# solislemuslab/BayesianNetworkRegression.jl

Measured on AMD Instinct MI355X. Metric: Gibbs iterations/sec (all chains), higher is better.
Workload: dtype f64; 1 GPU; synthetic n=500 V=100 (q=5050) R=7, 8 chains total, 8 per GPU; chains_total=8, chains_per_gpu=8, seed=20240501

## Files before the change

### bayesiannetworkregression.jl_amd/_capi.py

```python
import ctypes as C
import os

import numpy as np

from ._build import LIB

BNR_OK, BNR_ERR_BAD_ARG, BNR_ERR_HIP, BNR_ERR_CHOLESKY, BNR_ERR_SAMPLER = 0, 1, 2, 3, 4
BNR_ERR_SAMPLER_CAP = BNR_ERR_SAMPLER
ERRORS = {1: "bad argument", 2: "HIP error", 3: "Cholesky failed after jitter", 4: "sampler attempt cap"}


class BnrError(RuntimeError):
    def __init__(self, code, msg):
        super().__init__("libbnr_hip: %s (status %d: %s)" % (msg, code, ERRORS.get(code, "?")))
        self.code = code


class Hyper(C.Structure):
    _fields_ = [(k, C.c_double) for k in ("eta", "zeta", "iota", "aDelta", "bDelta", "nu")]


PROGRESS_CB = C.CFUNCTYPE(None, C.c_void_p, C.c_int64)
ALLGATHER_CB = C.CFUNCTYPE(C.c_int, C.c_void_p, C.POINTER(C.c_double), C.POINTER(C.c_double), C.c_int64)

# ... 36 lines not shown
    "bnr_chain_fetch": (C.c_int, [C.c_void_p, C.c_int32, C.c_int32, C.c_int32, C.c_int32] + [_dp] * 11),
    "bnr_chain_load": (C.c_int, [C.c_void_p, C.c_int32, C.c_int32, C.c_int32, C.c_int32] + [_dp] * 11),
    "bnr_chain_move_rows": (C.c_int, [C.c_void_p, C.c_int32, C.c_int32, C.c_int32]),
    "bnr_chain_resize": (C.c_int, [C.c_void_p, C.c_int32]),
    "bnr_chain_rhat_stats": (C.c_int, [C.c_void_p, C.c_int32, C.c_int32, _dp]),
    "bnr_chain_summary": (C.c_int, [C.c_void_p, C.c_int32, C.c_int32, C.c_int32, C.c_int32, _dp, _dp, _dp, _dp]),
    "bnr_chain_predict": (C.c_int, [C.c_void_p, C.c_int32, C.c_int32, C.c_int32, _dp, C.c_int32, _dp, C.c_int32, C.c_int32] + [_dp] * 5),
    "bnr_chain_predict_from_matrices": (C.c_int, [C.c_void_p, C.c_int32, C.c_int32, C.c_int32, C.POINTER(C.c_void_p), C.c_int32, _dp, C.c_int32,
                                                  C.c_int32] + [_dp] * 5),
    "bnr_chain_loglik_stats": (C.c_int, [C.c_void_p, C.c_int32, C.c_int32, _dp, _dp]),
    "bnr_chain_loo": (C.c_int, [C.c_void_p, C.c_int32, C.c_int32, _dp, _dp, _dp, _dp]),
    "bnr_psis_loo": (C.c_int, [C.c_int32, C.c_int32, C.c_int32, _dp, _dp, _dp, _dp, _dp]),
    "bnr_chains_summary": (C.c_int, [C.POINTER(C.c_void_p), C.c_int32, C.c_int32, C.c_int32, C.c_int32, C.c_int32, _dp, _dp, _dp, _dp]),
    "bnr_chains_predict": (C.c_int, [C.POINTER(C.c_void_p), C.c_int32, C.c_int32, C.c_int32, C.c_int32, _dp, C.c_int32, _dp, C.c_int32, C.c_int32]
                           + [_dp] * 5 + [C.c_uint64] + [_dp] * 3),
    "bnr_chains_predict_from_matrices": (C.c_int, [C.POINTER(C.c_void_p), C.c_int32, C.c_int32, C.c_int32, C.c_int32, C.POINTER(C.c_void_p), C.c_int32,
                                                   _dp, C.c_int32, C.c_int32] + [_dp] * 5 + [C.c_uint64] + [_dp] * 3),
    "bnr_chains_loglik_stats": (C.c_int, [C.POINTER(C.c_void_p), C.c_int32, C.c_int32, C.c_int32, _dp, _dp, _dp]),
    "bnr_chains_loo": (C.c_int, [C.POINTER(C.c_void_p), C.c_int32, C.c_int32, C.c_int32, _dp, _dp, _dp, _dp]),
    "bnr_chain_loo_predict": (C.c_int, [C.c_void_p, C.c_int32, C.c_int32, _dp, C.c_double, C.c_double] + [_dp] * 8),
    "bnr_chains_loo_predict": (C.c_int, [C.POINTER(C.c_void_p), C.c_int32, C.c_int32, C.c_int32, _dp, C.c_double, C.c_double] + [_dp] * 8),
    "bnr_psis_weights": (C.c_int, [C.c_int32, C.c_int32, C.c_int32, _dp, _dp, _dp, _dp, _dp]),
    "bnr_chain_rank_diag": (C.c_int, [C.c_void_p, C.c_int32, C.c_int32, C.c_int32] + [_dp] * 6),
    "bnr_chains_rank_diag": (C.c_int, [C.POINTER(C.c_void_p), C.c_int32, C.c_int32, C.c_int32, C.c_int32] + [_dp] * 6),
    "bnr_rank_normalize": (C.c_int, [C.c_int32, C.c_int32, C.c_int32, _dp, _dp, _dp]),
    "bnr_host_ndtri": (C.c_double, [C.c_double]),
    "bnr_chain_hdi": (C.c_int, [C.c_void_p, C.c_int32, C.c_int32, C.c_int32, _dp] + [_dp] * 5),
    "bnr_chains_hdi": (C.c_int, [C.POINTER(C.c_void_p), C.c_int32, C.c_int32, C.c_int32, C.c_int32, _dp] + [_dp] * 5),
    "bnr_hdi": (C.c_int, [C.c_int32, C.c_int32, C.c_int32, _dp, C.c_int32, _dp] + [_dp] * 5),
    "bnr_comm_unique_id": (C.c_int, [C.POINTER(UniqueId)]),
    "bnr_comm_create_rccl": (C.c_int, [C.POINTER(UniqueId), C.c_int32, C.c_int32, C.c_int32, C.POINTER(C.c_void_p)]),
    "bnr_comm_create_callback": (C.c_int, [C.c_int32, C.c_int32, ALLGATHER_CB, C.c_void_p, C.POINTER(C.c_void_p)]),
    "bnr_comm_destroy": (C.c_int, [C.c_void_p]),
    "bnr_comm_allgather": (C.c_int, [C.c_void_p, _dp, _dp, C.c_int64]),
    "bnr_comm_info": (C.c_int, [C.c_void_p] + [C.POINTER(C.c_int32)] * 5),
    "bnr_rhat": (C.c_int, [C.POINTER(C.c_void_p), C.c_int32, C.c_int32, C.c_void_p, C.c_int32, C.c_int32, _dp, _dp]),
    "bnr_rhat_from_stats": (C.c_int, [_dp, C.c_int32, C.c_int32, C.c_int32, _dp]),
    "bnr_chain_ess_stats": (C.c_int, [C.c_void_p, C.c_int32, C.c_int32, C.c_int32, _dp]),
    "bnr_ess_from_stats": (C.c_int, [_dp, C.c_int32, C.c_int32, C.c_int32, C.c_int32, _dp]),
    "bnr_chain_counters": (C.c_int, [C.c_void_p, C.POINTER(C.c_int64)]),
    "bnr_chain_set_profiling": (C.c_int, [C.c_void_p, C.c_int32]),
    "bnr_chain_last_timing": (C.c_int, [C.c_void_p, C.c_int32, C.POINTER(C.c_double), C.POINTER(C.c_int64)]),
    "bnr_chain_set_option": (C.c_int, [C.c_void_p, C.c_char_p, C.c_int64]),
    "bnr_chain_debug_read": (C.c_int, [C.c_void_p, C.POINTER(C.c_uint64), C.c_int32]),
    "bnr_chain_debug_copy": (C.c_int, [C.c_void_p, C.c_int32, _dp, C.c_int64]),
    "bnr_chain_debug_dims": (C.c_int, [C.c_void_p, C.POINTER(C.c_int32)]),
    "bnr_chain_debug_time_gram": (C.c_int, [C.c_void_p, C.c_int32, C.POINTER(C.c_double)]),
    "bnr_debug_set_exp": (C.c_int, [C.c_int32, C.c_int32]),
    "bnr_host_philox": (None, [C.POINTER(C.c_uint32), C.POINTER(C.c_uint32), C.POINTER(C.c_uint32)]),
    "bnr_host_uniform2": (None, [C.c_uint64, C.c_uint32, C.c_uint32, C.c_uint32, C.c_uint32, C.POINTER(C.c_double)]),
    "bnr_host_normal": (C.c_double, [C.c_uint64, C.c_uint32, C.c_uint32, C.c_uint32, C.c_uint32]),
    "bnr_host_gamma": (C.c_double, [C.c_uint64, C.c_double, C.c_uint32, C.c_uint32, C.c_uint32]),
    "bnr_host_gig": (C.c_double, [C.c_uint64, C.c_double, C.c_double, C.c_double, C.c_uint32, C.c_uint32]),
    "bnr_host_edge_index": (C.c_int32, [C.c_int32, C.c_int32, C.c_int32]),
    "bnr_host_xi_weight": (C.c_double, [C.c_double, C.c_double, C.c_double]),
    "bnr_host_pred_noise": (None, [C.c_uint64, C.c_uint32, C.c_uint32, C.c_uint32, C.c_uint32, _dp]),
    "bnr_host_gram_plan": (C.c_int, [C.c_int32, C.c_int32, C.c_int32, C.POINTER(C.c_int32)]),
}
for _u in ("tau2", "u_xi", "gamma", "D", "theta", "Delta", "M", "mu", "Lambda", "pi"):
    _SIGS["bnr_update_" + _u] = (C.c_int, [C.c_void_p, C.c_int32, C.c_int64])

EXPORTS = sorted(_SIGS)


_foreign_hip = None


def _mapped(needle):
    out = []
    try:
        with open("/proc/self/maps") as f:
            for line in f:
                parts = line.split()
                if len(parts) >= 6 and needle in os.path.basename(parts[5]) and parts[5] not in out:
                    out.append(parts[5])
    except OSError:
        pass
    return out


def lib():
    global _lib
    if _lib is None:
        if not os.path.exists(LIB):
            raise ImportError("libbnr_hip.so is missing at %s -- build it with `python -c 'import __graft_entry__ as g; "
                              "g.build()'` (hipcc --offload-arch=gfx950); there is no CPU fallback" % LIB)
        before = _mapped("libamdhip64")
        L = C.CDLL(LIB)
        after = _mapped("libamdhip64")
        foreign = [p_ for p_ in before if not os.path.realpath(p_).startswith(os.path.realpath(os.environ.get("ROCM_PATH", "/opt/rocm")))]
        global _foreign_hip
        if foreign and after == before and not os.environ.get("BNR_ALLOW_FOREIGN_HIP"):
            _foreign_hip = ("libbnr_hip.so was loaded after another HIP runtime (%s) and is bound to it instead of %s/lib: load the library "
                            "(bnr_amd._capi.lib(), or create the chains) BEFORE importing torch, or set BNR_ALLOW_FOREIGN_HIP=1 to run on the "
                            "foreign runtime" % (", ".join(foreign), os.environ.get("ROCM_PATH", "/opt/rocm")))
        for name, (res, args) in _SIGS.items():
            f = getattr(L, name)
            f.restype = res
            f.argtypes = args
        _lib = L
    return _lib


def check(code):
    if code != BNR_OK:
        raise BnrError(code, lib().bnr_last_error().decode())
# ... 631 lines not shown
```

### bayesiannetworkregression.jl_amd/csrc/bnr_hip.hip

```cpp
#include "bnr_internal.h"
#include "bnr_kernels.h"

#include <dlfcn.h>

#include <cmath>
#include <cstdio>
#include <mutex>

static thread_local std::string g_err;
int fail(int code, const std::string &msg) { g_err = msg; return code; }
static thread_local hipError_t g_noted = hipSuccess;
static thread_local const char *g_noted_what = nullptr;
#define HIPNOTE(expr)                                                                                  \
    do {                                                                                               \
        hipError_t _e = (expr);                                                                        \
        if (_e != hipSuccess && g_noted == hipSuccess) { g_noted = _e; g_noted_what = #expr; }         \
    } while (0)

template <typename T>
static int dev_alloc(bnr_chain *c, T **p, size_t count, bool zero = true)
{
    void *q = nullptr;
    HIPCHK(hipMalloc(&q, std::max<size_t>(count, 1) * sizeof(T)));
    if (zero) HIPCHK(hipMemsetAsync(q, 0, std::max<size_t>(count, 1) * sizeof(T), c->x.stream));
// ... 18 lines not shown
    std::lock_guard<std::mutex> lock(mu);
    if ((int)done.size() <= device) done.resize(device + 1, 0);
    if (done[device]) return BNR_OK;
    const int big = 124 * 1024;
    const void *fns[] = {(const void *)&k_tail<bnr_one>, (const void *)&k_tail<bnr_many>, (const void *)&k_backproj<bnr_one>,
                         (const void *)&k_backproj<bnr_many>, (const void *)&k_solve_a4<bnr_one>, (const void *)&k_solve_a4<bnr_many>,
                         (const void *)&k_xpass_group, (const void *)&k_node<bnr_one>, (const void *)&k_node<bnr_many>};
    for (const void *f : fns) HIPCHK(hipFuncSetAttribute(f, hipFuncAttributeMaxDynamicSharedMemorySize, big));
    if (int rc = late_kernels_lds_attributes(big)) return rc;
    done[device] = 1;
    return BNR_OK;
}

extern "C" {

static int exec_init(bnr_exec &x, int device, int nb, const bnr_dev *shape);
static void exec_free(bnr_exec &x);
static int sync_dev(bnr_chain *c);

int bnr_abi_version(void) { return BNR_ABI_VERSION; }
const char *bnr_last_error(void) { return g_err.c_str(); }
int bnr_device_synchronize(int32_t device)
{
    HIPCHK(hipSetDevice(device));
    HIPCHK(hipDeviceSynchronize());
    return BNR_OK;
}
int bnr_runtime_version(int *version)
{
    if (!version) return fail(BNR_ERR_BAD_ARG, "version is NULL");
    HIPCHK(hipRuntimeGetVersion(version));
    return BNR_OK;
}
int bnr_device_count(int *count)
{
    if (!count) return fail(BNR_ERR_BAD_ARG, "count is NULL");
    HIPCHK(hipGetDeviceCount(count));
    return BNR_OK;
}

void bnr_host_philox(const uint32_t ctr[4], const uint32_t key[2], uint32_t out[4])
{
    bnr_u4 r = bnr_philox4x32_10(ctr[0], ctr[1], ctr[2], ctr[3], key[0], key[1]);
    out[0] = r.x; out[1] = r.y; out[2] = r.z; out[3] = r.w;
}
void bnr_host_uniform2(uint64_t seed, uint32_t it, uint32_t site, uint32_t elem, uint32_t att, double out[2])
{ bnr_draw2(seed, it, site, elem, att, out[0], out[1]); }
double bnr_host_normal(uint64_t seed, uint32_t it, uint32_t site, uint32_t elem, uint32_t att)
{ return bnr_normal(seed, it, site, elem, att); }
double bnr_host_gamma(uint64_t seed, double shape, uint32_t it, uint32_t site, uint32_t elem)
{ int cap = 0; return bnr_gamma(seed, shape, it, site, elem, &cap); }
double bnr_host_gig(uint64_t seed, double lambda, double chi, double psi, uint32_t it, uint32_t elem)
{ int cap = 0; return bnr_gig(seed, lambda, chi, psi, it, elem, &cap); }
int32_t bnr_host_edge_index(int32_t V, int32_t l, int32_t k)
{ return l >= k ? bnr_edge_index(V, l, k) : bnr_edge_index(V, k, l); }
double bnr_host_xi_weight(double lt, double lb, double Delta)
{ return bnr_xi_weight_ref(lt, lb, Delta); }

static int alloc_trace(bnr_chain *c, int tot, double **out)
{
    void *p = nullptr;
    size_t bytes = (size_t)(tot + 2) * c->d.rowlen * sizeof(double);
    HIPCHK(hipMalloc(&p, bytes));
    HIPCHK(hipMemsetAsync(p, 0, bytes, c->x.stream));
    *out = (double *)p;
    c->trace_bytes = bytes;
    return BNR_OK;
}

extern "C++" size_t dtype_size(int t) { return t == BNR_U8 ? 1 : (t == BNR_I32 || t == BNR_F32) ? 4 : 8; }
extern "C++" template <typename T>
static void launch_x_convert_as(const void *raw, bool mats, int rows, const bnr_dev &d, int ld, double *Xd, unsigned char *X8, int *not_bytes, hipStream_t st)
{
    hipLaunchKernelGGL(k_x_convert<T>, dim3((rows + 63) / 64, std::min(d.q, 65535)), dim3(64), 0, st, (const T *)raw, mats, rows, d.V, d.q, ld, d.ek, d.el, Xd, X8,
                       not_bytes);
}
extern "C++" void launch_x_convert(int dtype, const void *raw, bool mats, int rows, const bnr_dev &d, int ld, double *Xd, unsigned char *X8, int *not_bytes, hipStream_t st)
{
    switch (dtype) {
    case BNR_U8:  launch_x_convert_as<uint8_t>(raw, mats, rows, d, ld, Xd, X8, not_bytes, st); break;
    case BNR_I32: launch_x_convert_as<int32_t>(raw, mats, rows, d, ld, Xd, X8, not_bytes, st); break;
    case BNR_I64: launch_x_convert_as<int64_t>(raw, mats, rows, d, ld, Xd, X8, not_bytes, st); break;
    case BNR_F32: launch_x_convert_as<float>(raw, mats, rows, d, ld, Xd, nullptr, not_bytes, st); break;
    default:      launch_x_convert_as<double>(raw, mats, rows, d, ld, Xd, nullptr, not_bytes, st); break;
    }
}
static int upload_x(bnr_chain *c, const x_source &src, double *Xd, unsigned char *X8, int *not_bytes_dev)
{
    const bnr_dev &d = c->d;
    const size_t es = dtype_size(src.dtype);
    if (!src.mats && src.dtype == BNR_F64) {
        HIPCHK(hipMemcpy2D(Xd, (size_t)d.n_pad * sizeof(double), src.X, (size_t)d.n * sizeof(double), (size_t)d.n * sizeof(double), d.q, hipMemcpyHostToDevice));
        return BNR_OK;
    }
    const size_t count = src.mats ? (size_t)d.n * d.V * d.V : (size_t)d.n * d.q;
    void *raw = nullptr;
    HIPCHK(hipMalloc(&raw, count * es));
    hipError_t e = hipSuccess;
    if (src.mats) {
        for (int i = 0; i < d.n && e == hipSuccess; ++i) {
            if (!src.mats[i]) { (void)hipFree(raw); return fail(BNR_ERR_BAD_ARG, "NULL adjacency matrix"); }
            e = hipMemcpyAsync((char *)raw + (size_t)i * d.V * d.V * es, src.mats[i], (size_t)d.V * d.V * es, hipMemcpyHostToDevice, c->x.stream);
        }
    } else e = hipMemcpyAsync(raw, src.X, count * es, hipMemcpyHostToDevice, c->x.stream);
    if (e == hipSuccess) {
        launch_x_convert(src.dtype, raw, src.mats != nullptr, d.n, d, d.n_pad, Xd, X8, not_bytes_dev, c->x.stream);
// ... 487 lines not shown
            BNR_CHOL_LAUNCHED();
            continue;
        }
        const int room = std::max(64, 2 * ncu - x.nb * npan);
        if (x.nb * ntile > room) {
            const int nsup = bnr_chol_nsuper(nbk, p);
            const int freecu = ncu - x.nb * npan;
            const int cap = p <= 4 ? 1 : x.spw_cap;
            const int spw = (freecu > 0 && nbk <= 24) ? std::min(cap, std::max(1, (x.nb * nsup + freecu - 1) / freecu)) : 1;
            if (few_ok && p >= 2) hipLaunchKernelGGL(HIP_KERNEL_NAME(k_chol_step<bnr_few>), dim3(x.nb, npan + (nsup + spw - 1) / spw), dim3(256), 0, st, few, p, s, 0, spw, fuse0);
            else BNR_LAUNCH(k_chol_step, dim3(x.nb, npan + (nsup + spw - 1) / spw), dim3(256), 0, st, x, p, s, 0, spw, fuse0);
        } else {
            if (few_ok && p >= 2) hipLaunchKernelGGL(HIP_KERNEL_NAME(k_chol_step<bnr_few>), dim3(x.nb, npan + ntile), dim3(256), 0, st, few, p, s, 1, 1, fuse0);
            else BNR_LAUNCH(k_chol_step, dim3(x.nb, npan + ntile), dim3(256), 0, st, x, p, s, 1, 1, fuse0);
        }
        BNR_CHOL_LAUNCHED();
    }
#undef BNR_CHOL_LAUNCHED
}
static int chol_launches(const bnr_exec &x)
{
    const int nbk = x.shape->n_pad / BNR_NB;
    return two_panel(x) ? nbk / 2 : nbk;
}
static double fact_est_us(const bnr_exec &x)
{
    const bool two_panel = chol_launches(x) != x.shape->n_pad / BNR_NB;
    return chol_launches(x) * (two_panel ? 18.5 : (x.nb > 1 ? 8.0 : 7.0));
}
static double scalar_est_us(const bnr_exec &x)
{
    return 45.0 + 0.0025 * x.shape->q * (x.nb > 1 ? 1.5 : 1.0) + 0.15 * x.shape->V * (x.nb > 1 ? 1.3 : 1.0);
}
static bool order_scalar_branch(const bnr_exec &x) { return x.overlap != 0 && fact_est_us(x) - scalar_est_us(x) >= 25.0; }
static int tail_after_default(const bnr_exec &x) { return order_scalar_branch(x) ? 0 : -1; }
static int node_after_default(const bnr_exec &x)
{
    if (!order_scalar_branch(x)) return -1;
    const double per = fact_est_us(x) / chol_launches(x);
    const int p = (int)((fact_est_us(x) - (scalar_est_us(x) - 20.0) - 20.0) / per);
    return std::max(0, std::min(p, chol_launches(x) / (x.nb > 1 ? 8 : 4)));
}
static int tail_after(const bnr_exec &x) { return x.tail_after == -2 ? tail_after_default(x) : x.tail_after; }
static int node_after(const bnr_exec &x) { const int v = x.node_after == -2 ? node_after_default(x) : x.node_after; return std::min(v, chol_launches(x) - 1); }
static void launch_solve(bnr_exec &x)
{
    BNR_LAUNCH(k_solve_w, dim3(x.shape->n_pad / 4, 1, x.nb), dim3(256), 0, x.stream, x);
    BNR_LAUNCH(k_solve_a4, dim3(x.shape->n_pad / BNR_NB, 1, x.nb), dim3(1024), (x.shape->n_pad + 32 * 33) * sizeof(double), x.stream, x);
}
static void launch_backproj(bnr_exec &x, int s, int flags)
{
    {
        const size_t lds64 = ((size_t)x.shape->n_pad + 64 + (size_t)x.shape->R * 65 + (size_t)(3 * x.shape->R + 1) * 65) * sizeof(double);
        const bool many_rounds = (size_t)x.nb * x.shape->nblk_bp >= (size_t)8 * x.ncu;
        if ((flags & 3) == 3 && lds64 <= 124 * 1024 && (x.wide_backproj == 1 || (x.wide_backproj < 0 && many_rounds))) {
            launch_late_backproj64(x, s, flags, lds64);
            return;
        }
    }
    size_t lds = std::max<size_t>(x.shape->n_pad + 64, (size_t)(3 * x.shape->R + 1) * 33) * sizeof(double);
    const int nslot = (x.nb * x.shape->nblk_bp <= 2 * x.ncu) ? 8 : 2;
    const int wide = (x.nb == 1 || x.shape->nblk_bp >= 1024) ? 256 : 0;
    BNR_LAUNCH(k_backproj, dim3(round_up(x.shape->nblk_bp, 8) * x.nb), dim3(256), lds, x.stream, x, s, flags | wide, x.nb, nslot);
}
static void launch_tail(bnr_exec &x, int s, int mask, int xg_src, unsigned wgs = 1)
{
    const size_t rv = (size_t)x.shape->R * x.shape->V;
    const size_t lds_a = (mask & BNR_TAIL_EARLY) ? tail_a_bytes(x) : 0;
    if (rv <= BNR_TAIL_U_LDS) { BNR_LAUNCH(k_tail, dim3(wgs, 1, x.nb), dim3(BNR_TAIL_THREADS), rv * sizeof(double) + lds_a, x.stream, x, s, mask, xg_src); return; }
    if (x.nb == 1) hipLaunchKernelGGL(HIP_KERNEL_NAME(k_tail<bnr_one, false>), dim3(wgs, 1, 1), dim3(BNR_TAIL_THREADS), lds_a, x.stream, bnr_one{*x.shape}, s, mask, xg_src);
    else hipLaunchKernelGGL(HIP_KERNEL_NAME(k_tail<bnr_many, false>), dim3(wgs, 1, x.nb), dim3(BNR_TAIL_THREADS), lds_a, x.stream, bnr_many{x.cds}, s, mask, xg_src);
}
static bool split_sums(const bnr_exec &x) { return x.split_sums == 1 || (x.split_sums < 0 && x.nb == 1 && x.shape->nblk_bp <= 3 * x.ncu && x.shape->n_pad >= 256); }
static void launch_full_tail(bnr_exec &x, int s)
{
    if (split_sums(x)) launch_backproj(x, s, 4);
    launch_tail(x, s, 1023, 0, 2);
}
static hipEvent_t next_event(bnr_exec &x)
{
    if (x.fj_next >= x.fj.size()) {
        hipEvent_t e = nullptr;
        HIPNOTE(hipEventCreateWithFlags(&e, hipEventDisableTiming));
        x.fj.push_back(e);
    }
    return x.fj[x.fj_next++];
}

static void launch_sweep(bnr_exec &x, int s, bool prev_tail)
{
    const bool timed = x.profiling != 0;
    const bool overlap = x.overlap != 0;
    hipStream_t sb = overlap ? x.stream2 : x.stream;
    hipEvent_t ej = nullptr;
    if (overlap) {
        hipEvent_t ef = next_event(x);
        HIPNOTE(hipEventRecord(ef, x.stream));
        HIPNOTE(hipStreamWaitEvent(x.stream2, ef, 0));
        launch_gram(x, s, sb, timed);
        hipEvent_t eg = nullptr, en = nullptr;
        if (tail_after(x) == 0 && prev_tail) { HIPNOTE(hipEventRecord(eg = next_event(x), x.stream2)); }
        if (node_after(x) >= 0) en = next_event(x);
        launch_chol(x, s, sb, node_after(x), en);
        HIPNOTE(hipEventRecord(ej = next_event(x), x.stream2));
        if (eg) HIPNOTE(hipStreamWaitEvent(x.stream, eg, 0));
        if (prev_tail) launch_full_tail(x, s - 1);
        if (en) HIPNOTE(hipStreamWaitEvent(x.stream, en, 0));
    } else
// ... 1232 lines not shown
```

### bayesiannetworkregression.jl_amd/csrc/bnr_kernels.h

```cpp
#pragma once
#include "bnr_device.h"

#define BNR_RMAX 32
#define BNR_NB 32
#define BNR_GT 64


#define BNR_GLOBAL_PTR(member) d.member = (decltype(d.member))(__attribute__((address_space(1))) void *)(unsigned long long)(d.member)
__device__ __forceinline__ bnr_dev bnr_globalized(const bnr_dev *src)
{
    bnr_dev d = *src;
    BNR_GLOBAL_PTR(X); BNR_GLOBAL_PTR(X8); BNR_GLOBAL_PTR(XM); BNR_GLOBAL_PTR(Sdig); BNR_GLOBAL_PTR(y); BNR_GLOBAL_PTR(ek); BNR_GLOBAL_PTR(el); BNR_GLOBAL_PTR(trace); BNR_GLOBAL_PTR(plan);
    BNR_GLOBAL_PTR(pbase); BNR_GLOBAL_PTR(Wbuf); BNR_GLOBAL_PTR(sz); BNR_GLOBAL_PTR(PW); BNR_GLOBAL_PTR(PA); BNR_GLOBAL_PTR(PG);
    BNR_GLOBAL_PTR(Gpart); BNR_GLOBAL_PTR(E); BNR_GLOBAL_PTR(gmap); BNR_GLOBAL_PTR(a3); BNR_GLOBAL_PTR(xw); BNR_GLOBAL_PTR(a4);
    BNR_GLOBAL_PTR(res); BNR_GLOBAL_PTR(xg); BNR_GLOBAL_PTR(bw); BNR_GLOBAL_PTR(wv); BNR_GLOBAL_PTR(scal); BNR_GLOBAL_PTR(Minv);
    BNR_GLOBAL_PTR(Psum); BNR_GLOBAL_PTR(counters); BNR_GLOBAL_PTR(dbg); BNR_GLOBAL_PTR(stamp); BNR_GLOBAL_PTR(gprog); BNR_GLOBAL_PTR(gmapc); BNR_GLOBAL_PTR(dfctl);
    return d;
}
struct bnr_one {
    bnr_dev d;
    __device__ __forceinline__ const bnr_dev &get() const { return d; }
    __device__ __forceinline__ const bnr_dev &get_x() const { return d; }
    __device__ __forceinline__ const bnr_dev &at(int) const { return d; }
};
// ... 2761 lines not shown
    case 2: bnr_xg_columns<2>(xp, ld, ne, sWZ, aw, aa); break;
    case 3: bnr_xg_columns<3>(xp, ld, ne, sWZ, aw, aa); break;
    case 4: bnr_xg_columns<4>(xp, ld, ne, sWZ, aw, aa); break;
    case 5: bnr_xg_columns<5>(xp, ld, ne, sWZ, aw, aa); break;
    case 6: bnr_xg_columns<6>(xp, ld, ne, sWZ, aw, aa); break;
    case 7: bnr_xg_columns<7>(xp, ld, ne, sWZ, aw, aa); break;
    default: bnr_xg_columns<8>(xp, ld, ne, sWZ, aw, aa); break;
    }
}
template <int LATE>
__global__ __launch_bounds__(256) void k_xpass_group2(const bnr_many chain_src, int s, int nchains)
{
    extern __shared__ double sh[];
    const int wg = blockIdx.x;
    const bnr_dev &c0 = chain_src.at(0);
    const int rs = (c0.n_pad + 255) / 256, bid = wg / rs, slice = wg % rs, tid = threadIdx.x;
    const int chunk = c0.chunk_x, e0 = bid * chunk, ne = min(chunk, c0.q - e0), R = c0.R;
    const size_t ld = c0.n_pad;
    double *sWZ = sh;
    __shared__ double *s_pw[8], *s_pa[8];
    const int i = slice * 256 + tid;
    const bool live = i < c0.n_pad;
    const int ic = live ? i : 0;
    for (int cb = 0; cb < nchains; cb += 8) {
        const int nc = min(8, nchains - cb);
        __syncthreads();
        for (int it = tid; it < nc * chunk; it += 256) {
            const int c = it / chunk, t = it - c * chunk;
            const bnr_dev &cd = chain_src.at(cb + c);
            const bnr_plan_entry P = cd.plan[cd.pbase[0] + s];
            const double *row = cd.trace + (size_t)P.row * cd.rowlen, *prev = cd.trace + (size_t)P.prev * cd.rowlen;
            double w = 0.0, zz = 0.0;
            if (t < ne) {
                const int e = e0 + t;
                w = edge_W(row + cd.o_u, prev + cd.o_lam, R, cd.el[e], cd.ek[e]);
                zz = sqrt(prev[cd.o_S + e]) * bnr_normal(cd.seed, P.it, SITE_G_Z1, (uint32_t)e, 0);
                if (slice == 0) { cd.Wbuf[e] = w; cd.sz[e] = zz; }
            }
            sWZ[(size_t)t * 16 + 2 * c] = w; sWZ[(size_t)t * 16 + 2 * c + 1] = zz;
        }
        if (tid < nc) { const bnr_dev &cd = chain_src.at(cb + tid); s_pw[tid] = cd.PW; s_pa[tid] = cd.PA; }
        __syncthreads();
        double aw[8], aa[8];
#pragma unroll
        for (int c = 0; c < 8; ++c) { aw[c] = 0.0; aa[c] = 0.0; }
        if (c0.X8) bnr_xg_dispatch(nc, c0.X8 + (size_t)e0 * ld + ic, ld, ne, sWZ, aw, aa);
        else bnr_xg_dispatch(nc, c0.X + (size_t)e0 * ld + ic, ld, ne, sWZ, aw, aa);
#pragma unroll
        for (int c = 0; c < 8; ++c)
            if (c < nc && live) { s_pw[c][(size_t)bid * ld + i] = aw[c]; s_pa[c][(size_t)bid * ld + i] = aa[c]; }
    }
}

template <class SRC>
__global__ __launch_bounds__(256) void k_backproj64(const SRC chain_src, int s, int flags, int nchains)
{
    BNR_CRITICAL_PATH();
    const int gid = blockIdx.x, gx = gid & 7, gr = gid >> 3;
    const int pid = (gr / nchains) * 8 + gx;
    const bnr_dev &cd = chain_src.at(gr % nchains);
    if (2 * pid >= cd.nblk_bp) return;
    const int R = cd.R, n_pad = cd.n_pad, nterm = 1 + 3 * R;
    extern __shared__ double sh[];
    double *sa = sh, *sdot = sa + n_pad, *sdr = sdot + 64, *st = sdr + R * 65;
    const bnr_plan_entry P = cd.plan[cd.pbase[0] + s];
    double *row = cd.trace + (size_t)P.row * cd.rowlen;
    const double *prev = cd.trace + (size_t)P.prev * cd.rowlen;
    const int tid = threadIdx.x, wave = tid >> 6, lane = tid & 63;
    const int e0 = pid * 64, ne = min(64, cd.q - e0);
    const size_t ld = cd.n_pad;
    const double tau2 = row[ROW_TAU2], tau = sqrt(tau2), psi = prev[ROW_THETA];
    if (flags & 4) {
        const double *un0 = row + cd.o_u;
        for (int idx = tid; idx < R * 64; idx += 256) {
            const int r = idx >> 6, ee = idx & 63;
            double v = 0.0;
            if (ee < ne) { const int l0 = cd.el[e0 + ee], k0 = cd.ek[e0 + ee]; v = un0[r + R * l0] * un0[r + R * k0]; }
            sdr[r * 65 + ee] = v;
        }
    }
    for (int i = tid; i < n_pad; i += 256) sa[i] = cd.a4[i];
    __syncthreads();
    for (int t = wave; t < ne; t += 16) {
        const int t2 = t + 4, t3 = t + 8, t4 = t + 12;
        const size_t oc = (size_t)(e0 + t) * ld, od = (size_t)(e0 + (t2 < ne ? t2 : t)) * ld, oe = (size_t)(e0 + (t3 < ne ? t3 : t)) * ld, of = (size_t)(e0 + (t4 < ne ? t4 : t)) * ld;
        double acc0 = 0.0, acc1 = 0.0, acc2 = 0.0, acc3 = 0.0;
        if (cd.X8) {
            const unsigned char *xc = cd.X8 + oc, *xd = cd.X8 + od, *xe = cd.X8 + oe, *xf = cd.X8 + of;
#pragma unroll 4
            for (int i = lane; i < n_pad; i += 64) { double av = sa[i]; acc0 = fma((double)xc[i], av, acc0); acc1 = fma((double)xd[i], av, acc1); acc2 = fma((double)xe[i], av, acc2); acc3 = fma((double)xf[i], av, acc3); }
        } else {
            const double *xc = cd.X + oc, *xd = cd.X + od, *xe = cd.X + oe, *xf = cd.X + of;
#pragma unroll 4
            for (int i = lane; i < n_pad; i += 64) { double av = sa[i]; acc0 = fma(xc[i], av, acc0); acc1 = fma(xd[i], av, acc1); acc2 = fma(xe[i], av, acc2); acc3 = fma(xf[i], av, acc3); }
        }
        acc0 = wave_sum(acc0); acc1 = wave_sum(acc1); acc2 = wave_sum(acc2); acc3 = wave_sum(acc3);
        if (lane == 0) { sdot[t] = acc0; if (t2 < ne) sdot[t2] = acc1; if (t3 < ne) sdot[t3] = acc2; if (t4 < ne) sdot[t4] = acc3; }
    }
    __syncthreads();
    if (wave != (pid & 3)) return;
    const int e = e0 + lane;
    const bool act = lane < ne;
    int cap = 0;
    double gam = 0.0, W = 0.0, Snew = 1.0;
    if (act) {
        W = cd.Wbuf[e];
        const double Sp = prev[cd.o_S + e];
        gam = tau * (cd.sz[e] + Sp * sdot[lane]) + W;
        row[cd.o_gamma + e] = gam;
        const double g = gam - W, chi = (g * g) / tau2;
        Snew = bnr_gig(cd.seed, 0.5, chi, psi, P.it, (uint32_t)e, &cap);
        row[cd.o_S + e] = Snew;
    }
    if (cap) atomicAdd((unsigned long long *)&cd.counters[2], 1ull);
    if (!(flags & 4)) return;
    const double sd = sqrt(tau2 * Snew), lsd = log(sd) + 0.5 * log(2.0 * BNR_PI);
    const double *lamp = prev + cd.o_lam;
    st[lane] = act ? Snew : 0.0;
    for (int r = 0; r < R; ++r) {
        const double dr = sdr[r * 65 + lane], lr = lamp[r];
#pragma unroll
        for (int c = 0; c < 3; ++c) {
            const double Wc = W + (bnr_lambda_value(c) - lr) * dr;
            const double zz = (gam - Wc) / sd;
            st[(1 + 3 * r + c) * 65 + lane] = act ? (-0.5 * zz * zz - lsd) : 0.0;
        }
    }
    bnr_wsync();
    const int half = lane >> 5, chunk = 2 * pid + half;
    if (chunk < cd.nblk_bp) {
        double *ps = cd.Psum + (size_t)chunk * nterm;
        for (int j = lane & 31; j < nterm; j += 32) {
            double acc = 0.0;
#pragma unroll 8
            for (int e2 = 0; e2 < 32; ++e2) acc += st[j * 65 + 32 * half + e2];
            ps[j] = acc;
        }
    }
}

template <class SRC, int L>
__global__ __launch_bounds__(1024) void k_sdigits(const SRC chain_src, int s)
{
    const bnr_dev &cd = chain_src.get_x();
    const int tid = threadIdx.x;
    const bnr_plan_entry P = cd.plan[cd.pbase[0] + s];
    const double *S = cd.trace + (size_t)P.prev * cd.rowlen + cd.o_S;
    __shared__ double red[16];
    __shared__ int s_nonfinite;
    if (tid == 0) s_nonfinite = 0;
    __syncthreads();
    double m = 0.0, m1 = 0.0, m2 = 0.0, m3 = 0.0;
    int k = tid;
    for (; k + 3072 < cd.q; k += 4096) { m = fmax(m, S[k]); m1 = fmax(m1, S[k + 1024]); m2 = fmax(m2, S[k + 2048]); m3 = fmax(m3, S[k + 3072]); }
    for (; k < cd.q; k += 1024) m = fmax(m, S[k]);
    {
        double z = 0.0;
        for (int kk2 = tid; kk2 < cd.q; kk2 += 1024) { const double v = S[kk2]; z += v - v; }
        if (!(z == 0.0)) atomicOr(&s_nonfinite, 1);
    }
    m = fmax(fmax(m, m1), fmax(m2, m3));
    m = fmax(m, __shfl_xor(m, 32)); m = fmax(m, __shfl_xor(m, 16)); m = fmax(m, __shfl_xor(m, 8));
    m = fmax(m, __shfl_xor(m, 4)); m = fmax(m, __shfl_xor(m, 2)); m = fmax(m, __shfl_xor(m, 1));
    if ((tid & 63) == 0) red[tid >> 6] = m;
    __syncthreads();
    m = red[0];
    for (int w = 1; w < 16; ++w) m = fmax(m, red[w]);
    if (s_nonfinite) {
        if (tid == 0) bnr_flag_gfail(cd);
        m = 1.0;
    }
    int e;
    (void)frexp(m, &e);
    constexpr int BITS = 8 * L - 2;
    const double up = ldexp(1.0, BITS - e);
    if (tid == 0 && blockIdx.y == 0) cd.scal[SC_I8SCALE] = ldexp(1.0, e - BITS);
    const int kchunk = cd.q_pad / cd.ksplit;
    for (int idx = (int)blockIdx.y * 1024 + tid; idx < cd.kslab; idx += (int)gridDim.y * 1024) {
        const int ks = idx / cd.kcp, kk = idx % cd.kcp, k = ks * kchunk + kk;
        unsigned long long N = 0;
        if (kk < kchunk && k < cd.q && !s_nonfinite) N = (unsigned long long)(S[k] * up + 0.5);
        unsigned carry = 0;
#pragma unroll
        for (int l = L - 1; l >= 0; --l) {
            const unsigned b = (unsigned)((N >> (8 * (L - 1 - l))) & 255ull) + carry;
            carry = b >= 128u ? 1u : 0u;
            cd.Sdig[(size_t)l * cd.kslab + idx] = (unsigned char)(b & 255u);
        }
    }
// ... 2 lines not shown
```

### include/bnr_hip.h

```cpp
#ifndef BNR_HIP_H
#define BNR_HIP_H

#include <stdint.h>

#ifdef __cplusplus
extern "C" {
#endif

#define BNR_ABI_VERSION 13

enum {
    BNR_OK = 0,
    BNR_ERR_BAD_ARG = 1,
    BNR_ERR_HIP = 2,
    BNR_ERR_CHOLESKY = 3,
    BNR_ERR_SAMPLER_CAP = 4
};

typedef struct bnr_chain bnr_chain;

typedef struct {
    double eta, zeta, iota, aDelta, bDelta, nu;
} bnr_hyper;

typedef void (*bnr_progress_cb)(void *user, int64_t done);

int bnr_abi_version(void);
const char *bnr_last_error(void);
int bnr_device_count(int *count);
int bnr_device_synchronize(int32_t device);
int bnr_runtime_version(int *version);

int bnr_chain_create(int32_t n, int32_t V, int32_t R, const double *X, const double *y, const bnr_hyper *hyper,
                     uint64_t seed, int32_t chain_id, int32_t device, int32_t tot_save, bnr_chain **out);
enum { BNR_F64 = 0, BNR_U8 = 1 , BNR_I32 = 2, BNR_I64 = 3 , BNR_F32 = 4 };
int bnr_chain_create_typed(int32_t n, int32_t V, int32_t R, const void *X, int32_t x_dtype, const double *y, const bnr_hyper *hyper,
                           uint64_t seed, int32_t chain_id, int32_t device, int32_t tot_save, bnr_chain **out);
int bnr_chain_create_from_matrices(int32_t n, int32_t V, int32_t R, const void *const *A, int32_t x_dtype, const double *y,
                                   const bnr_hyper *hyper, uint64_t seed, int32_t chain_id, int32_t device, int32_t tot_save,
                                   bnr_chain **out);
int bnr_chain_create_like(const bnr_chain *donor, uint64_t seed, int32_t chain_id, int32_t tot_save, bnr_chain **out);
int bnr_chain_destroy(bnr_chain *chain);

int bnr_chain_init_prior(bnr_chain *chain);

int bnr_chain_run(bnr_chain *chain, int32_t first_index, int32_t nburn, int32_t total, int32_t purge_burn,
                  int32_t prog_freq, bnr_progress_cb cb, void *user, int32_t *next_row);
int bnr_chain_run_async(bnr_chain *chain, int32_t first_index, int32_t nburn, int32_t total, int32_t purge_burn);
int bnr_chain_sync(bnr_chain *chain, int32_t *next_row);
int bnr_chain_prepare(bnr_chain *chain);

typedef struct bnr_group bnr_group;
int bnr_group_create(bnr_chain *const *chains, int32_t nchains, bnr_group **out);
int bnr_group_destroy(bnr_group *group);
int bnr_group_run(bnr_group *group, int32_t first_index, int32_t nburn, int32_t total, int32_t purge_burn,
                  int32_t prog_freq, bnr_progress_cb cb, void *user, int32_t *next_row);
int bnr_group_prepare(bnr_group *group);
int bnr_group_set_option(bnr_group *group, const char *name, int64_t value);
int bnr_group_last_timing(bnr_group *group, int32_t which, double *avg_us, int64_t *launches);

int bnr_gibbs_step(bnr_chain *chain, int32_t row, int64_t iter);
int bnr_update_tau2(bnr_chain *chain, int32_t row, int64_t iter);
// ... 54 lines not shown
                           double p_hi, double *lpd, double *elpd_loo, double *pareto_k, double *loo_mean, double *loo_sd, double *loo_pit,
                           double *loo_lower, double *loo_upper);
int bnr_psis_weights(int32_t device, int32_t m, int32_t nsamp, const double *loglik, const double *r_eff, double *log_weights, double *elpd_loo,
                     double *pareto_k);

int bnr_chain_rank_diag(bnr_chain *chain, int32_t first_row, int32_t nsamp, int32_t max_lag, double *rhat_bulk, double *rhat_tail,
                        double *ess_bulk, double *ess_tail, double *ess_mean, double *mcse_mean);
int bnr_chains_rank_diag(bnr_chain *const *chains, int32_t nchains, int32_t first_row, int32_t nsamp, int32_t max_lag, double *rhat_bulk,
                         double *rhat_tail, double *ess_bulk, double *ess_tail, double *ess_mean, double *mcse_mean);
int bnr_rank_normalize(int32_t device, int32_t m, int32_t S, const double *x, double *ranks, double *z);

int bnr_chain_hdi(bnr_chain *chain, int32_t first_row, int32_t nsamp, int32_t nprob, const double *probs, double *lower, double *upper,
                  double *median, double *p_pos, double *p_neg);
int bnr_chains_hdi(bnr_chain *const *chains, int32_t nchains, int32_t first_row, int32_t nsamp, int32_t nprob, const double *probs, double *lower,
                   double *upper, double *median, double *p_pos, double *p_neg);
int bnr_hdi(int32_t device, int32_t m, int32_t S, const double *x, int32_t nprob, const double *probs, double *lower, double *upper, double *median,
            double *p_pos, double *p_neg);

int bnr_chain_ess_stats(bnr_chain *chain, int32_t first_row, int32_t nsamp, int32_t max_lag, double *stats);
int bnr_ess_from_stats(const double *stats, int32_t nchains, int32_t nparams, int32_t nsamp, int32_t max_lag, double *ess);

typedef struct bnr_comm bnr_comm;
typedef struct { char bytes[128]; } bnr_unique_id;
typedef int (*bnr_allgather_fn)(void *ctx, const double *send, double *recv, int64_t count);
int bnr_comm_unique_id(bnr_unique_id *id);
int bnr_comm_create_rccl(const bnr_unique_id *id, int32_t rank, int32_t world, int32_t device, bnr_comm **out);
int bnr_comm_create_callback(int32_t rank, int32_t world, bnr_allgather_fn fn, void *ctx, bnr_comm **out);
int bnr_comm_destroy(bnr_comm *comm);
int bnr_comm_allgather(bnr_comm *comm, const double *send, double *recv, int64_t count);
int bnr_comm_info(bnr_comm *comm, int32_t *kind, int32_t *rank, int32_t *world, int32_t *rccl_ranks, int32_t *rccl_rank);
int bnr_rhat(bnr_chain *const *chains, int32_t nchains_local, int32_t nchains_total, bnr_comm *comm, int32_t burn, int32_t nsamp,
             double *rhat_xi, double *rhat_gamma);

int bnr_rhat_from_stats(const double *stats, int32_t nchains, int32_t nparams, int32_t nsamp, double *rhat);

int bnr_chain_counters(bnr_chain *chain, int64_t out[8]);

int bnr_chain_set_profiling(bnr_chain *chain, int32_t enable);
int bnr_chain_last_timing(bnr_chain *chain, int32_t which, double *avg_us, int64_t *launches);

int bnr_chain_debug_read(bnr_chain *chain, uint64_t *out, int32_t count);
int bnr_chain_debug_time_gram(bnr_chain *chain, int32_t reps, double *avg_us);
int bnr_chain_debug_copy(bnr_chain *chain, int32_t which, double *out, int64_t count);
int bnr_chain_debug_dims(bnr_chain *chain, int32_t *out8);
int bnr_debug_set_exp(int32_t device, int32_t flags);

int bnr_chain_set_option(bnr_chain *chain, const char *name, int64_t value);

void bnr_host_philox(const uint32_t ctr[4], const uint32_t key[2], uint32_t out[4]);
void bnr_host_uniform2(uint64_t seed, uint32_t it, uint32_t site, uint32_t elem, uint32_t att, double out[2]);
double bnr_host_normal(uint64_t seed, uint32_t it, uint32_t site, uint32_t elem, uint32_t att);
double bnr_host_gamma(uint64_t seed, double shape, uint32_t it, uint32_t site, uint32_t elem);
double bnr_host_gig(uint64_t seed, double lambda, double chi, double psi, uint32_t it, uint32_t elem);
int32_t bnr_host_edge_index(int32_t V, int32_t l, int32_t k);
void bnr_host_pred_noise(uint64_t seed, uint32_t s0, uint32_t ns, uint32_t i0, uint32_t ni, double *out);
double bnr_host_ndtri(double p);
double bnr_host_xi_weight(double lt, double lb, double Delta);
int bnr_host_gram_plan(int32_t n, int32_t V, int32_t ncu, int32_t out[4]);

#ifdef __cplusplus
}
#endif
#endif
```

Before: 22000 iterations/s.

## Parallelize GIG rejection retries across lanes and split kinds over two waves

In the wide backprojection kernel, the GIG draw for S now splits by sampler kind across two waves instead of running on one. Lanes still open after the first rejection attempt are compacted into shared memory and retried with several lanes per element, each trying a different attempt index. This cuts divergence-driven serial retry loops. The per-rank log-likelihood terms and the partial-sum reduction are spread across all four waves, and the wide-kernel selection heuristic now favors the wide path when multiple chains are batched. It adds static LDS use, extra block syncs, and a host helper that counts attempts for testing.

After: 22300 iterations/s (median of 6 runs). 1.01x the previous value.

```diff
diff --git a/bayesiannetworkregression.jl_amd/_capi.py b/bayesiannetworkregression.jl_amd/_capi.py
--- a/bayesiannetworkregression.jl_amd/_capi.py
+++ b/bayesiannetworkregression.jl_amd/_capi.py
@@ -112,6 +112,7 @@
     "bnr_host_normal": (C.c_double, [C.c_uint64, C.c_uint32, C.c_uint32, C.c_uint32, C.c_uint32]),
     "bnr_host_gamma": (C.c_double, [C.c_uint64, C.c_double, C.c_uint32, C.c_uint32, C.c_uint32]),
     "bnr_host_gig": (C.c_double, [C.c_uint64, C.c_double, C.c_double, C.c_double, C.c_uint32, C.c_uint32]),
+    "bnr_host_gig_attempts": (C.c_int32, [C.c_uint64, C.c_double, C.c_double, C.c_double, C.c_uint32, C.c_uint32]),
     "bnr_host_edge_index": (C.c_int32, [C.c_int32, C.c_int32, C.c_int32]),
     "bnr_host_xi_weight": (C.c_double, [C.c_double, C.c_double, C.c_double]),
     "bnr_host_pred_noise": (None, [C.c_uint64, C.c_uint32, C.c_uint32, C.c_uint32, C.c_uint32, _dp]),
diff --git a/bayesiannetworkregression.jl_amd/csrc/bnr_hip.hip b/bayesiannetworkregression.jl_amd/csrc/bnr_hip.hip
--- a/bayesiannetworkregression.jl_amd/csrc/bnr_hip.hip
+++ b/bayesiannetworkregression.jl_amd/csrc/bnr_hip.hip
@@ -94,6 +94,17 @@
 { int cap = 0; return bnr_gamma(seed, shape, it, site, elem, &cap); }
 double bnr_host_gig(uint64_t seed, double lambda, double chi, double psi, uint32_t it, uint32_t elem)
 { int cap = 0; return bnr_gig(seed, lambda, chi, psi, it, elem, &cap); }
+int32_t bnr_host_gig_attempts(uint64_t seed, double lambda, double chi, double psi, uint32_t it, uint32_t elem)
+{
+    bnr_gig_ctx c;
+    bnr_gig_setup(c, lambda, chi, psi);
+    if (c.kind != 2 && c.kind != 3) return -1;
+    for (uint32_t k = 0; k < BNR_MAX_ATTEMPTS; ++k) {
+        double out;
+        if (bnr_gig_try(c, seed, it, elem, k, out)) return (int32_t)k;
+    }
+    return (int32_t)BNR_MAX_ATTEMPTS;
+}
 int32_t bnr_host_edge_index(int32_t V, int32_t l, int32_t k)
 { return l >= k ? bnr_edge_index(V, l, k) : bnr_edge_index(V, k, l); }
 double bnr_host_xi_weight(double lt, double lb, double Delta)
@@ -687,8 +698,9 @@
 {
     {
         const size_t lds64 = ((size_t)x.shape->n_pad + 64 + (size_t)x.shape->R * 65 + (size_t)(3 * x.shape->R + 1) * 65) * sizeof(double);
-        const bool many_rounds = (size_t)x.nb * x.shape->nblk_bp >= (size_t)8 * x.ncu;
-        if ((flags & 3) == 3 && lds64 <= 124 * 1024 && (x.wide_backproj == 1 || (x.wide_backproj < 0 && many_rounds))) {
+        const size_t chunks = (size_t)x.nb * x.shape->nblk_bp;
+        const bool many_rounds = x.nb > 1 ? chunks > (size_t)x.ncu : chunks >= (size_t)8 * x.ncu;
+        if ((flags & 3) == 3 && lds64 + BNR_BP64_STATIC_LDS <= 124 * 1024 && (x.wide_backproj == 1 || (x.wide_backproj < 0 && many_rounds))) {
             launch_late_backproj64(x, s, flags, lds64);
             return;
         }
diff --git a/bayesiannetworkregression.jl_amd/csrc/bnr_kernels.h b/bayesiannetworkregression.jl_amd/csrc/bnr_kernels.h
--- a/bayesiannetworkregression.jl_amd/csrc/bnr_kernels.h
+++ b/bayesiannetworkregression.jl_amd/csrc/bnr_kernels.h
@@ -2837,6 +2837,73 @@
     }
 }
 
+#define BNR_BP_NF 11
+#define BNR_BP64_STATIC_LDS ((2 * BNR_BP_NF * 64 + 3 * 64) * sizeof(double) + 2 * 64 * sizeof(int))
+template <int KIND>
+__device__ __forceinline__ void bnr_bp_stage(double (*sc)[64], int slot, const bnr_gig_ctx &c)
+{
+    sc[0][slot] = c.alpha; sc[1][slot] = c.xm;
+    if (KIND == 2) { sc[2][slot] = c.ulo; sc[3][slot] = c.uhi; sc[4][slot] = c.xoff; sc[5][slot] = c.t; sc[6][slot] = c.s; sc[7][slot] = c.nc; }
+    else { sc[2][slot] = c.omega; sc[3][slot] = c.Atot; sc[4][slot] = c.A0; sc[5][slot] = c.A1; sc[6][slot] = c.x0; sc[7][slot] = c.k0; sc[8][slot] = c.k1; sc[9][slot] = c.k2; sc[10][slot] = c.x0l; }
+}
+template <int KIND>
+__device__ __forceinline__ void bnr_bp_unstage(bnr_gig_ctx &c, const double (*sc)[64], int slot, double lambda)
+{
+    c.kind = KIND; c.lambda_old = lambda; c.lambda = lambda < 0.0 ? -lambda : lambda; c.half = (c.lambda == 0.5) ? 1 : 0;
+    c.alpha = sc[0][slot]; c.xm = sc[1][slot];
+    if (KIND == 2) { c.ulo = sc[2][slot]; c.uhi = sc[3][slot]; c.xoff = sc[4][slot]; c.t = sc[5][slot]; c.s = sc[6][slot]; c.nc = sc[7][slot]; }
+    else { c.omega = sc[2][slot]; c.Atot = sc[3][slot]; c.A0 = sc[4][slot]; c.A1 = sc[5][slot]; c.x0 = sc[6][slot]; c.k0 = sc[7][slot]; c.k1 = sc[8][slot]; c.k2 = sc[9][slot]; c.x0l = sc[10][slot]; }
+}
+template <int KIND>
+__device__ __forceinline__ double bnr_bp_draw(bool mine, double chi, double psi, uint64_t seed, uint32_t it, int e0, int lane, double (*sc)[64], double *sres, int *sopen, int *cap)
+{
+    double Snew = 1.0;
+    bool open = false;
+    bnr_gig_ctx c;
+    if (mine) {
+        bnr_gig_setup(c, 0.5, chi, psi);
+        c.kind = KIND;
+        double out;
+        if (bnr_gig_try(c, seed, it, (uint32_t)(e0 + lane), 0u, out)) Snew = out; else open = true;
+    }
+    const unsigned long long om = __ballot(open), below = (1ull << lane) - 1ull;
+    int m = __popcll(om);
+    if (m == 0) return Snew;
+    if (open) { bnr_bp_stage<KIND>(sc, lane, c); sopen[__popcll(om & below)] = lane; }
+    bnr_wsync();
+    uint32_t base = 1u;
+    while (m > 0 && base < BNR_MAX_ATTEMPTS) {
+        const int lg = m <= 4 ? 4 : (m <= 8 ? 3 : (m <= 16 ? 2 : (m <= 32 ? 1 : 0))), A = 1 << lg;
+        const int j = lane >> lg, a = lane & (A - 1);
+        const uint32_t k = base + (uint32_t)a;
+        const bool has = j < m;
+        const int src = has ? sopen[j] : 0;
+        if (has) bnr_bp_unstage<KIND>(c, sc, src, 0.5);
+        double out = 0.0;
+        const bool ok = has && k < BNR_MAX_ATTEMPTS && bnr_gig_try(c, seed, it, (uint32_t)(e0 + src), k, out);
+        const unsigned grp = (unsigned)(__ballot(ok) >> (j << lg)) & ((1u << A) - 1u);
+        if (ok && a == __ffs(grp) - 1) sres[src] = out;
+        const bool still = has && a == 0 && grp == 0u;
+        const unsigned long long sm = __ballot(still);
+        bnr_wsync();
+        if (still) sopen[__popcll(sm & below)] = src;
+        m = __popcll(sm);
+        base += (uint32_t)A;
+        bnr_wsync();
+    }
+    if (m > 0) {
+        if (lane < m) {
+            const int src = sopen[lane];
+            bnr_bp_unstage<KIND>(c, sc, src, 0.5);
+            if (cap) *cap = 1;
+            sres[src] = c.alpha * c.xm;
+        }
+        bnr_wsync();
+    }
+    if (open) Snew = sres[lane];
+    return Snew;
+}
+
 template <class SRC>
 __global__ __launch_bounds__(256) void k_backproj64(const SRC chain_src, int s, int flags, int nchains)
 {
@@ -2883,26 +2950,44 @@
         if (lane == 0) { sdot[t] = acc0; if (t2 < ne) sdot[t2] = acc1; if (t3 < ne) sdot[t3] = acc2; if (t4 < ne) sdot[t4] = acc3; }
     }
     __syncthreads();
-    if (wave != (pid & 3)) return;
+    __shared__ double s_ctx[2][BNR_BP_NF][64];
+    __shared__ double s_res[2][64], s_S[64];
+    __shared__ int s_open[2][64];
+    const int w2 = pid & 3, w3 = (pid + 2) & 3;
     const int e = e0 + lane;
     const bool act = lane < ne;
-    int cap = 0;
-    double gam = 0.0, W = 0.0, Snew = 1.0;
+    double gam = 0.0, W = 0.0;
     if (act) {
         W = cd.Wbuf[e];
         const double Sp = prev[cd.o_S + e];
         gam = tau * (cd.sz[e] + Sp * sdot[lane]) + W;
-        row[cd.o_gamma + e] = gam;
+        if (wave == w2) row[cd.o_gamma + e] = gam;
+    }
+    if (wave == w2 || wave == w3) {
+        int cap = 0;
         const double g = gam - W, chi = (g * g) / tau2;
-        Snew = bnr_gig(cd.seed, 0.5, chi, psi, P.it, (uint32_t)e, &cap);
-        row[cd.o_S + e] = Snew;
-    }
-    if (cap) atomicAdd((unsigned long long *)&cd.counters[2], 1ull);
+        const int kind = act ? bnr_gig_kind(0.5, chi, psi) : -1;
+        if (wave == w2) {
+            double Snew = bnr_bp_draw<2>(kind == 2, chi, psi, cd.seed, P.it, e0, lane, s_ctx[0], s_res[0], s_open[0], &cap);
+            if (act && kind != 2 && kind != 3) {
+                bnr_gig_ctx gc;
+                bnr_gig_setup(gc, 0.5, chi, psi);
+                Snew = bnr_gig_degenerate(gc, cd.seed, chi, psi, P.it, (uint32_t)e, &cap);
+            }
+            if (kind != 3) { s_S[lane] = Snew; if (act) row[cd.o_S + e] = Snew; }
+        } else {
+            const double Snew = bnr_bp_draw<3>(kind == 3, chi, psi, cd.seed, P.it, e0, lane, s_ctx[1], s_res[1], s_open[1], &cap);
+            if (kind == 3) { s_S[lane] = Snew; row[cd.o_S + e] = Snew; }
+        }
+        if (cap) atomicAdd((unsigned long long *)&cd.counters[2], 1ull);
+    }
     if (!(flags & 4)) return;
+    __syncthreads();
+    const double Snew = s_S[lane];
     const double sd = sqrt(tau2 * Snew), lsd = log(sd) + 0.5 * log(2.0 * BNR_PI);
     const double *lamp = prev + cd.o_lam;
-    st[lane] = act ? Snew : 0.0;
-    for (int r = 0; r < R; ++r) {
+    if (wave == w2) st[lane] = act ? Snew : 0.0;
+    for (int r = wave; r < R; r += 4) {
         const double dr = sdr[r * 65 + lane], lr = lamp[r];
 #pragma unroll
         for (int c = 0; c < 3; ++c) {
@@ -2911,15 +2996,14 @@
             st[(1 + 3 * r + c) * 65 + lane] = act ? (-0.5 * zz * zz - lsd) : 0.0;
         }
     }
-    bnr_wsync();
-    const int half = lane >> 5, chunk = 2 * pid + half;
-    if (chunk < cd.nblk_bp) {
-        double *ps = cd.Psum + (size_t)chunk * nterm;
-        for (int j = lane & 31; j < nterm; j += 32) {
+    __syncthreads();
+    for (int idx = tid; idx < 2 * nterm; idx += 256) {
+        const int half = idx >= nterm ? 1 : 0, j = idx - half * nterm, chunk = 2 * pid + half;
+        if (chunk < cd.nblk_bp) {
             double acc = 0.0;
 #pragma unroll 8
             for (int e2 = 0; e2 < 32; ++e2) acc += st[j * 65 + 32 * half + e2];
-            ps[j] = acc;
+            cd.Psum[(size_t)chunk * nterm + j] = acc;
         }
     }
 }
diff --git a/include/bnr_hip.h b/include/bnr_hip.h
--- a/include/bnr_hip.h
+++ b/include/bnr_hip.h
@@ -7,7 +7,7 @@
 extern "C" {
 #endif
 
-#define BNR_ABI_VERSION 13
+#define BNR_ABI_VERSION 14
 
 enum {
     BNR_OK = 0,
@@ -168,6 +168,7 @@
 double bnr_host_normal(uint64_t seed, uint32_t it, uint32_t site, uint32_t elem, uint32_t att);
 double bnr_host_gamma(uint64_t seed, double shape, uint32_t it, uint32_t site, uint32_t elem);
 double bnr_host_gig(uint64_t seed, double lambda, double chi, double psi, uint32_t it, uint32_t elem);
+int32_t bnr_host_gig_attempts(uint64_t seed, double lambda, double chi, double psi, uint32_t it, uint32_t elem);
 int32_t bnr_host_edge_index(int32_t V, int32_t l, int32_t k);
 void bnr_host_pred_noise(uint64_t seed, uint32_t s0, uint32_t ns, uint32_t i0, uint32_t ni, double *out);
 double bnr_host_ndtri(double p);
```
